# indutny/elliptic

Hardware: NVIDIA H100
Metric: secp256k1 ECDSA verifies/sec (higher is better)
Workload: dtype u32 limbs (integer, exact)

## Files before the change

elliptic_b200/csrc/eb200.cu:

```cuda
#include <cuda_runtime.h>
#include <stdio.h>
#include <string.h>
#include <atomic>
#include <condition_variable>
#include <cstdlib>
#include <mutex>
#include <thread>
#include <type_traits>
#include <vector>
#include "../../include/elliptic_b200.h"
#include "ecdsa_k256_body.cuh"
#include "ecdsa_k256_replay.cuh"
#include "ecdsa_sw_replay.cuh"
#include "ecdsa_k256_sign_fast.cuh"
#include "der_sig.cuh"
#include "ecdsa_sw_sign.cuh"
#include "ecdsa_k256_sign.cuh"
#include "ecdsa_sw_body.cuh"
#include "ed25519_body.cuh"
#include "ed25519_ec.cuh"
#include "sw_runtime.cuh"

using namespace eb;

#ifndef EB_VERIFY_BLOCK
#define EB_VERIFY_BLOCK 128
#endif
#ifndef EB_VERIFY_MINBLOCKS
#define EB_VERIFY_MINBLOCKS 3
#endif

__global__ void __launch_bounds__(128) k256_gtab_kernel(u32* gtab) {
  size_t t = (size_t)blockIdx.x * blockDim.x + threadIdx.x;
  if (t >= (size_t)GTAB_WINDOWS * GTAB_ENTRIES) return;
  int j = (int)(t / GTAB_ENTRIES), idx = (int)(t % GTAB_ENTRIES);
  gtab_entry(j, idx, gtab + t * 16);
}

__global__ void __launch_bounds__(128) k256_prep_kernel(size_t N, const uint8_t* __restrict__ e,
                                                        const uint8_t* __restrict__ r,
                                                        const uint8_t* __restrict__ s,
                                                        u32* __restrict__ ws, u32* __restrict__ scratch) {
  size_t tid = (size_t)blockIdx.x * blockDim.x + threadIdx.x;
  size_t T = (size_t)gridDim.x * blockDim.x;
  prep_thread(tid, T, N, e, r, s, ws, scratch);
}

__global__ void __launch_bounds__(EB_VERIFY_BLOCK, EB_VERIFY_MINBLOCKS)
k256_verify_kernel(size_t N, const uint8_t* __restrict__ pub, const uint8_t* __restrict__ r,
                   const u32* __restrict__ ws, const u32* __restrict__ gtab,
                   u32* __restrict__ qtab, const uint8_t* __restrict__ pre, uint8_t* __restrict__ status) {
  size_t i = (size_t)blockIdx.x * blockDim.x + threadIdx.x;
  if (i >= N) return;
  if (pre && pre[i]) { status[i] = pre[i]; return; }
  status[i] = verify_item(i, N, pub, r, ws, gtab, qtab);
}

__global__ void __launch_bounds__(128) k256_prep_recover_kernel(size_t N, const uint8_t* __restrict__ e,
                                                                const uint8_t* __restrict__ r,
                                                                const uint8_t* __restrict__ s,
                                                                u32* __restrict__ ws, u32* __restrict__ scratch) {
  size_t tid = (size_t)blockIdx.x * blockDim.x + threadIdx.x;
  size_t T = (size_t)gridDim.x * blockDim.x;
  prep_thread(tid, T, N, e, r, s, ws, scratch, 1);
}
__global__ void __launch_bounds__(EB_VERIFY_BLOCK, EB_VERIFY_MINBLOCKS)
k256_recover_kernel(size_t N, const uint8_t* __restrict__ r, const uint8_t* __restrict__ recid,
                    const u32* __restrict__ ws, const u32* __restrict__ gtab, u32* __restrict__ qtab,
                    uint8_t* __restrict__ out, uint8_t* __restrict__ status) {
  size_t i = (size_t)blockIdx.x * blockDim.x + threadIdx.x;
  if (i >= N) return;
  status[i] = recover_item(i, N, r, recid, ws, gtab, qtab, out);
}

__global__ void __launch_bounds__(128)
k256_sign_nonce_kernel(size_t N, const uint8_t* __restrict__ e, const uint8_t* __restrict__ priv,
                       const u32* __restrict__ gtab, u32* __restrict__ ws, uint8_t* __restrict__ status,
                       const uint8_t* __restrict__ kgiven) {
  size_t i = (size_t)blockIdx.x * blockDim.x + threadIdx.x;
  if (i < N) k256_sign_nonce_item(i, N, e, priv, gtab, ws, status, kgiven);
}
__global__ void __launch_bounds__(128)
k256_sign_finish_kernel(size_t N, const uint8_t* __restrict__ e, const uint8_t* __restrict__ priv, u32 canonical,
                        const u32* __restrict__ ws, u32* __restrict__ scratch, uint8_t* __restrict__ r,
                        uint8_t* __restrict__ s, uint8_t* __restrict__ recid, uint8_t* __restrict__ status) {
  size_t tid = (size_t)blockIdx.x * blockDim.x + threadIdx.x;
  size_t T = (size_t)gridDim.x * blockDim.x;
  k256_sign_finish_thread(tid, T, N, e, priv, canonical, ws, scratch, r, s, recid, status);
}
__global__ void __launch_bounds__(128)
k256_sign_slow_kernel(size_t N, const uint8_t* __restrict__ e, const uint8_t* __restrict__ priv, u32 canonical,
                      const u32* __restrict__ gtab, uint8_t* __restrict__ r, uint8_t* __restrict__ s,
                      uint8_t* __restrict__ recid, uint8_t* __restrict__ status) {
  size_t i = (size_t)blockIdx.x * blockDim.x + threadIdx.x;
  if (i >= N || status[i] != ST_NEEDS_HOST) return;
  status[i] = k256_sign_item(i, e, priv, canonical, gtab, r, s, recid);
}

__global__ void __launch_bounds__(128) k256_replay_tab_kernel(u32* tab) {
  int t = blockIdx.x * blockDim.x + threadIdx.x;
  if (t < 2 * REPLAY_NAF_PTS) rp_tab_entry(t, tab + 16 * t);
}
__global__ void __launch_bounds__(128)
k256_replay_kernel(size_t N, const uint8_t* __restrict__ e, const uint8_t* __restrict__ r, const uint8_t* __restrict__ s,
                   const uint8_t* __restrict__ pub, const u32* __restrict__ tab, uint8_t* __restrict__ status) {
  size_t i = (size_t)blockIdx.x * blockDim.x + threadIdx.x;
  if (i >= N || status[i] != ST_NEEDS_HOST) return;
  status[i] = rp_verify_item(i, e, r, s, pub, tab);
}

__global__ void __launch_bounds__(128)
k256_prep_scalars_kernel(size_t N, const uint8_t* __restrict__ k1, const uint8_t* __restrict__ k2, u32* __restrict__ ws) {
  size_t i = (size_t)blockIdx.x * blockDim.x + threadIdx.x;
  if (i < N) prep_scalars_item(i, N, k1, k2, ws);
}
__global__ void __launch_bounds__(EB_VERIFY_BLOCK, EB_VERIFY_MINBLOCKS)
k256_mul_add_kernel(size_t N, const uint8_t* __restrict__ pts, const u32* __restrict__ ws, const u32* __restrict__ gtab,
                    u32* __restrict__ qtab, uint8_t* __restrict__ out, uint8_t* __restrict__ status) {
  size_t i = (size_t)blockIdx.x * blockDim.x + threadIdx.x;
  if (i >= N) return;
  status[i] = mul_add_item(i, N, pts, ws, gtab, qtab, out);
}
__global__ void __launch_bounds__(128)
k256_mul_add_replay_kernel(size_t N, const uint8_t* __restrict__ k1, const uint8_t* __restrict__ k2,
                           const uint8_t* __restrict__ pts, const u32* __restrict__ tab, uint8_t* __restrict__ out,
                           uint8_t* __restrict__ status) {
  size_t i = (size_t)blockIdx.x * blockDim.x + threadIdx.x;
  if (i >= N || status[i] != ST_NEEDS_HOST) return;
  status[i] = rp_mul_add_item(i, k1, k2, pts, tab, out);
}
__global__ void __launch_bounds__(128)
k256_mul_g_kernel(size_t N, const uint8_t* __restrict__ k, const u32* __restrict__ gtab, uint8_t* __restrict__ out,
                  uint8_t* __restrict__ status) {
  size_t i = (size_t)blockIdx.x * blockDim.x + threadIdx.x;
  if (i >= N) return;
  status[i] = k256_mul_g_item(i, k, gtab, out);
}

__global__ void status_map_kernel(size_t N, uint8_t* __restrict__ status, uint8_t from, uint8_t to) {
  size_t i = (size_t)blockIdx.x * blockDim.x + threadIdx.x;
  if (i < N && status[i] == from) status[i] = to;
}

__global__ void __launch_bounds__(128)
der_decode_kernel(size_t N, u32 len, const uint8_t* __restrict__ der, const unsigned long long* __restrict__ off,
                  uint8_t* __restrict__ r, uint8_t* __restrict__ s, uint8_t* __restrict__ pre, int pre_valid) {
  size_t i = (size_t)blockIdx.x * blockDim.x + threadIdx.x;
  if (i >= N) return;
  bool ok = der_import(der + off[i], (size_t)(off[i + 1] - off[i]), len, r + (size_t)len * i, s + (size_t)len * i);
  uint8_t st = pre_valid ? pre[i] : 0;
  if (!st && !ok) st = ST_THROW_SIG_FORMAT;
  pre[i] = st;
}

__global__ void __launch_bounds__(128) k256_decode_pub_kernel(size_t N, const uint8_t* __restrict__ in, u32 fmt,
                                                              uint8_t* __restrict__ xy, uint8_t* __restrict__ pre) {
  size_t i = (size_t)blockIdx.x * blockDim.x + threadIdx.x;
  if (i >= N) return;
  uint8_t st = 0;
  if (fmt == EB200_PUB_SEC1_65) {
    const uint8_t* p = in + 65 * i;
    uint8_t tag = p[0];
    if (tag != 4 && tag != 6 && tag != 7) st = ST_THROW_POINT_FORMAT;
    else if ((tag == 6 && (p[64] & 1)) || (tag == 7 && !(p[64] & 1))) st = ST_THROW_ASSERT;
    for (int k = 0; k < 64; k++) xy[64 * i + k] = p[1 + k];
  } else {
    const uint8_t* p = in + 33 * i;
    uint8_t tag = p[0];
    if (tag != 2 && tag != 3) st = ST_THROW_POINT_FORMAT;
    fe x = fe_from_be(p + 1);
    fe seven = fe_zero(); seven.v[0] = 7;
    fe y2 = fe_add(fe_mul(fe_sqr(x), x), seven);
    fe y = fe_sqrt_candidate(y2);
    if (!st && !fe_eq(fe_sqr(y), y2)) st = ST_THROW_INVALID_POINT;
    y = fe_normalize(y);
    bool odd = tag == 3;
    if (((y.v[0] & 1) != 0) != odd) y = fe_normalize(fe_neg(y));
    x = fe_normalize(x);
    store_be<8>(xy + 64 * i, x.v);
    store_be<8>(xy + 64 * i + 32, y.v);
  }
  pre[i] = st;
// ... 1674 lines not shown
```

elliptic_b200/csrc/ecdsa_k256_body.cuh:

```cuda
#pragma once
#include "ge_k256.cuh"
#include "sc_k256.cuh"
#ifndef EB_K256_FQ
#define EB_K256_FQ 0
#endif
#include "gq_k256.cuh"

namespace eb {

enum : uint8_t {
  ST_FALSE = 0, ST_TRUE = 1, ST_THROW_INVALID_POINT = 2, ST_THROW_NOT_VALIDATED = 3,
  ST_NEEDS_HOST = 4, ST_THROW_ASSERT = 5, ST_THROW_POINT_FORMAT = 6, ST_INFINITY = 7, ST_THROW_SECOND_KEY = 8, ST_THROW_SIG_FORMAT = 9,
};

constexpr int PREP_WORDS = 19;
constexpr u32 FL_INVALID = 1, FL_NEGG = 2, FL_NEG1 = 4, FL_NEG2 = 8, FL_NOG = 16;
constexpr int PREP_BATCH = 16;
constexpr int QTAB_ENTRIES = 8;
#if EB_K256_FQ
constexpr int QTAB_WORDS = QTABQ_WORDS;
#else
constexpr int QTAB_WORDS = QTAB_ENTRIES * 24;
#endif
#ifndef EB_GW
#define EB_GW 20
#endif
constexpr int GTAB_W = EB_GW;
constexpr int GTAB_WINDOWS = (255 + GTAB_W - 1) / GTAB_W;
constexpr int GTAB_ENTRIES = 1 << (GTAB_W - 1);
static_assert(255 - GTAB_W * (GTAB_WINDOWS - 1) <= GTAB_W - 1, "top digit 2m+1 must stay below 2^W");

struct madd_out { ge_jac r; fe h; };

#if defined(__CUDACC__)
#define EB_FN __host__ __device__ __noinline__
#else
#define EB_FN
#endif

EB_FN ge_jac jac_dbl(ge_jac p) { return jac_dbl_inl(p); }
EB_FN ge_jac jac_madd(ge_jac a, ge_aff p) { return jac_madd_inl(a, p); }

EB_HD madd_out jac_madd_h(const ge_jac& a, const ge_aff& p) {
  madd_out o;
  fe z2 = fe_sqr(a.z);
  fe u2 = fe_mul(p.x, z2);
  fe s2 = fe_mul(fe_mul(p.y, z2), a.z);
  fe h = fe_sub(a.x, u2);
  fe rr = fe_sub(a.y, s2);
  fe h2 = fe_sqr(h);
  fe h3 = fe_mul(h2, h);
  fe v = fe_mul(a.x, h2);
  o.r.x = fe_sub(fe_sub(fe_add(fe_sqr(rr), h3), v), v);
  o.r.y = fe_sub(fe_mul(rr, fe_sub(v, o.r.x)), fe_mul(a.y, h3));
  o.r.z = fe_mul(a.z, h);
  o.h = h;
  return o;
}

EB_HD fe fe_beta() {
  fe b;
  const u32 v[8] = {0x719501eeu, 0xc1396c28u, 0x12f58995u, 0x9cf04975u, 0xac3434e9u, 0x6e64479eu, 0x657c0710u, 0x7ae96a2bu};
  for (int i = 0; i < 8; i++) b.v[i] = v[i];
  return b;
}

EB_HD ge_aff k256_G() {
  ge_aff g;
  const u32 x[8] = {0x16f81798u, 0x59f2815bu, 0x2dce28d9u, 0x029bfcdbu, 0xce870b07u, 0x55a06295u, 0xf9dcbbacu, 0x79be667eu};
  const u32 y[8] = {0xfb10d4b8u, 0x9c47d08fu, 0xa6855419u, 0xfd17b448u, 0x0e1108a8u, 0x5da4fbfcu, 0x26a3c465u, 0x483ada77u};
  for (int i = 0; i < 8; i++) { g.x.v[i] = x[i]; g.y.v[i] = y[i]; }
  return g;
}

EB_HD void gtab_entry(int j, int idx, u32* out16) {
  ge_jac b = jac_from_aff(k256_G());
  for (int k = 0; k < GTAB_W * j; k++) b = jac_dbl(b);
  ge_aff base = jac_to_aff(b);
  u32 s = 2 * idx + 1;
  ge_jac acc = jac_infinity();
  for (int k = GTAB_W - 1; k >= 0; k--) {
    acc = jac_dbl(acc);
    if ((s >> k) & 1) acc = jac_madd(acc, base);
  }
  ge_aff r = jac_to_aff(acc);
  r.x = fe_normalize(r.x);
  r.y = fe_normalize(r.y);
  for (int i = 0; i < 8; i++) { out16[i] = r.x.v[i]; out16[8 + i] = r.y.v[i]; }
}

EB_HD void prep_store(size_t i, size_t N, u32* u1, const u32* u2, u32 flags, u32* ws) {
  u32 nn[8];
  K256N::n(nn);
  if ((u1[0] & 1) == 0) {
    sub_n<8>(u1, nn, u1);
    flags |= FL_NEGG;
  }
  u32 m1[5], m2[5];
  bool n1, n2;
  glv_split_odd(u2, m1, &n1, m2, &n2);
  if (n1) flags |= FL_NEG1;
  if (n2) flags |= FL_NEG2;
  for (int w = 0; w < 8; w++) {
    u32 hi = (w < 7) ? u1[w + 1] : 0;
    ws[(size_t)w * N + i] = (u1[w] >> 1) | (hi << 31);
  }
  for (int w = 0; w < 5; w++) {
    ws[(size_t)(8 + w) * N + i] = m1[w];
    ws[(size_t)(13 + w) * N + i] = m2[w];
  }
  ws[(size_t)18 * N + i] = flags;
}

EB_HD void prep_thread(size_t tid, size_t T, size_t N, const uint8_t* e, const uint8_t* r,
                       const uint8_t* s, u32* ws, u32* scratch, int mode = 0) {
  u32 R2[8], one[8], nn[8];
  K256N::r2(R2); K256N::r1(one); K256N::n(nn);
  u32 prod[8];
  copy_n<8>(prod, one);
  u32 invalid_mask = 0;
  int cnt = 0;
  for (int j = 0; j < PREP_BATCH; j++) {
    size_t i = tid + (size_t)j * T;
    if (i >= N) break;
    cnt = j + 1;
    u32 sv[8], rv[8];
    load_be<8>(sv, s + 32 * i);
    load_be<8>(rv, r + 32 * i);
    bool ok = sc_in_range(sv) && sc_in_range(rv);
    u32 sm[8];
    if (mode == 1) {
      sc_mont_mul(sm, rv, R2);
      ok = !is_zero_n<8>(sm);
    } else {
      sc_mont_mul(sm, sv, R2);
    }
    if (!ok) invalid_mask |= 1u << j;
    cmov_n<8>(sm, one, !ok);
    for (int w = 0; w < 8; w++) scratch[(size_t)w * N + i] = prod[w];
    u32 t[8];
    sc_mont_mul(t, prod, sm);
    copy_n<8>(prod, t);
  }
  if (cnt == 0) return;
  u32 inv[8];
  sc_mont_inv(inv, prod);
  for (int j = cnt - 1; j >= 0; j--) {
    size_t i = tid + (size_t)j * T;
    bool ok = !((invalid_mask >> j) & 1);
    u32 sv[8], rv[8], ev[8], sm[8], pre[8], sinv[8], t[8];
    load_be<8>(sv, s + 32 * i);
    load_be<8>(rv, r + 32 * i);
    sc_mont_mul(sm, mode == 1 ? rv : sv, R2);
    cmov_n<8>(sm, one, !ok);
    for (int w = 0; w < 8; w++) pre[w] = scratch[(size_t)w * N + i];
    sc_mont_mul(sinv, inv, pre);
    sc_mont_mul(t, inv, sm);
    copy_n<8>(inv, t);
    u32 flags = (ok || mode == 1) ? 0 : FL_INVALID;
    load_be<8>(ev, e + 32 * i);
    u32 u1[8], u2[8];
    if (mode == 1) {
      u32 zero8[8] = {0, 0, 0, 0, 0, 0, 0, 0};
      cmov_n<8>(sinv, zero8, !ok);
      sc_mont_mul(u1, ev, sinv);
      if (!is_zero_n<8>(u1)) sub_n<8>(u1, nn, u1);
      sc_mont_mul(u2, sv, sinv);
    } else {
      sc_mont_mul(u1, ev, sinv);
      sc_mont_mul(u2, rv, sinv);
    }
    prep_store(i, N, u1, u2, flags, ws);
  }
}

EB_HD void prep_scalars_item(size_t i, size_t N, const uint8_t* k1, const uint8_t* k2, u32* ws) {
  u32 nn[8], u1[8] = {0, 0, 0, 0, 0, 0, 0, 0}, u2[8];
  K256N::n(nn);
  u32 flags = 0;
  if (k1) {
    load_be<8>(u1, k1 + 32 * i);
    if (geq_n<8>(u1, nn)) sub_n<8>(u1, u1, nn);
  } else {
    flags |= FL_NOG;
  }
  load_be<8>(u2, k2 + 32 * i);
  if (geq_n<8>(u2, nn)) sub_n<8>(u2, u2, nn);
  prep_store(i, N, u1, u2, flags, ws);
}

EB_HD void store_fe(u32* dst, const fe& a) { for (int i = 0; i < 8; i++) dst[i] = a.v[i]; }
EB_HD fe load_fe(const u32* src) { fe a; for (int i = 0; i < 8; i++) a.v[i] = src[i]; return a; }

#if EB_K256_FQ
EB_HD ge_jac k256_dsm(size_t i, size_t N, const ge_aff& Q, u32 flags, const u32* ws, const u32* gtab, u32* qtab) {
  u32* tab = qtab + (size_t)i * QTAB_WORDS;
  fqk<1> zglobal;
  {
    gq_jac Qj; Qj.x = fqk_from_fe(Q.x); Qj.y = fqk_from_fe(Q.y); Qj.z = fqk_one();
    gq_jac D = gq_dbl(Qj);
    fqk<1> C2 = fq_sqr(D.z);
    fqk<1> C3 = fq_mul(C2, D.z);
    gq_jac P;
    P.x = fq_mul(Qj.x, C2);
    P.y = fq_mul(Qj.y, C3);
    P.z = fqk_one();
    fq_store12(tab + 0, P.x); fq_store12(tab + FQ_PAD, P.y);
    for (int k = 1; k < QTAB_ENTRIES; k++) {
      gq_madd_out o = gq_madd_h(P, D.x, D.y);
      P = o.r;
      u32* e = tab + QTABQ_ENTRY_WORDS * k;
      fq_store12(e, P.x); fq_store12(e + FQ_PAD, P.y);
      fq_store12(e + 2 * FQ_PAD, o.h);
    }
    zglobal = fq_mul(P.z, D.z);
    const fqk<1> beta = fqk_from_fe(fe_beta());
    fqk<1> zs = fqk_one();
    for (int k = QTAB_ENTRIES - 1; k >= 0; k--) {
      u32* e = tab + QTABQ_ENTRY_WORDS * k;
      fqk<1> X = fq_load12(e), Y = fq_load12(e + FQ_PAD);
      fqk<1> hk = fqk_one();
      if (k > 0) hk = fq_load12(e + 2 * FQ_PAD);
      if (k < QTAB_ENTRIES - 1) {
        fqk<1> zs2 = fq_sqr(zs);
        fqk<1> zs3 = fq_mul(zs2, zs);
        X = fq_mul(X, zs2);
        Y = fq_mul(Y, zs3);
        fq_store12(e, X); fq_store12(e + FQ_PAD, Y);
      }
      fq_store12(e + 2 * FQ_PAD, fq_mul(X, beta));
      zs = fq_mul(zs, hk);
    }
  }

  gq_jac acc;
  acc.x = fqk_one(); acc.y = fqk_one(); acc.z = fqk_zero();
  for (int w = 32; w >= 0; w--) {
    if (w != 32)
      for (int d = 0; d < 4; d++) acc = gq_dbl(acc);
    for (int h = 0; h < 2; h++) {
      u32 word = ws[(size_t)((h ? 13 : 8) + (w >> 3)) * N + i];
      u32 nib = (word >> (4 * (w & 7))) & 15;
      bool dneg = (w != 32) && (nib < 8);
      u32 idx = (w == 32) ? (nib & 7) : (dneg ? 7 - nib : nib - 8);
      bool neg = dneg != (((flags & (h ? FL_NEG2 : FL_NEG1)) != 0));
      const u32* e = tab + QTABQ_ENTRY_WORDS * idx;
      gq_aff P;
      P.x = fq_load12(e + (h ? 2 * FQ_PAD : 0));
      P.y = fq_cneg(fq_load12(e + FQ_PAD), neg);
      if (w == 32 && h == 0) acc = gq_from_aff(P);
      else acc = gq_madd(acc, P);
    }
  }
  acc.z = fq_mul(acc.z, zglobal);

  if (!(flags & FL_NOG)) {
    for (int j = 0; j < GTAB_WINDOWS; j++) {
      const int pos = GTAB_W * j;
      u32 lo = ws[(size_t)(pos >> 5) * N + i];
      u32 hi = ((pos >> 5) < 7) ? ws[(size_t)((pos >> 5) + 1) * N + i] : 0u;
      u64 both = ((u64)hi << 32) | lo;
      u32 chunk = (u32)(both >> (pos & 31)) & ((1u << GTAB_W) - 1);
      const u32 half = 1u << (GTAB_W - 1);
      bool dneg = (j != GTAB_WINDOWS - 1) && (chunk < half);
      u32 idx = (j == GTAB_WINDOWS - 1) ? (chunk & (half - 1)) : (dneg ? half - 1 - chunk : chunk - half);
      bool neg = dneg != ((flags & FL_NEGG) != 0);
      const u32* ent = gtab + ((size_t)j * GTAB_ENTRIES + idx) * 16;
      gq_aff P;
      P.x = fqk_from_fe(load_fe(ent));
      P.y = fq_cneg(fqk_from_fe(load_fe(ent + 8)), neg);
      acc = gq_madd(acc, P);
    }
  }
  return gq_to_jac(acc);
}
#else
EB_HD ge_jac k256_dsm(size_t i, size_t N, const ge_aff& Q, u32 flags, const u32* ws, const u32* gtab, u32* qtab) {
  u32* tab = qtab + (size_t)i * QTAB_WORDS;
  fe zglobal;
  {
    ge_jac D = jac_dbl(jac_from_aff(Q));
    fe C2 = fe_sqr(D.z);
    fe C3 = fe_mul(C2, D.z);
    ge_aff Dp; Dp.x = D.x; Dp.y = D.y;
    ge_jac P;
    P.x = fe_mul(Q.x, C2);
    P.y = fe_mul(Q.y, C3);
    P.z = fe_one();
    store_fe(tab + 0, P.x); store_fe(tab + 8, P.y);
    for (int k = 1; k < QTAB_ENTRIES; k++) {
      madd_out o = jac_madd_h(P, Dp);
      P = o.r;
      store_fe(tab + 24 * k, P.x); store_fe(tab + 24 * k + 8, P.y);
      store_fe(tab + 24 * k + 16, o.h);
    }
    zglobal = fe_mul(P.z, D.z);
    fe beta = fe_beta();
    fe zs = fe_one();
    for (int k = QTAB_ENTRIES - 1; k >= 0; k--) {
      fe X = load_fe(tab + 24 * k), Y = load_fe(tab + 24 * k + 8);
      fe hk = fe_one();
      if (k > 0) hk = load_fe(tab + 24 * k + 16);
      if (k < QTAB_ENTRIES - 1) {
        fe zs2 = fe_sqr(zs);
        fe zs3 = fe_mul(zs2, zs);
        X = fe_mul(X, zs2);
        Y = fe_mul(Y, zs3);
        store_fe(tab + 24 * k, X); store_fe(tab + 24 * k + 8, Y);
      }
      store_fe(tab + 24 * k + 16, fe_mul(X, beta));
      zs = fe_mul(zs, hk);
    }
  }

  ge_jac acc = jac_infinity();
  for (int w = 32; w >= 0; w--) {
    if (w != 32)
      for (int d = 0; d < 4; d++) acc = jac_dbl(acc);
    for (int h = 0; h < 2; h++) {
      u32 word = ws[(size_t)((h ? 13 : 8) + (w >> 3)) * N + i];
      u32 nib = (word >> (4 * (w & 7))) & 15;
      bool dneg = (w != 32) && (nib < 8);
      u32 idx = (w == 32) ? (nib & 7) : (dneg ? 7 - nib : nib - 8);
      bool neg = dneg != (((flags & (h ? FL_NEG2 : FL_NEG1)) != 0));
      ge_aff P;
      P.x = load_fe(tab + 24 * idx + (h ? 16 : 0));
      P.y = load_fe(tab + 24 * idx + 8);
      P = aff_neg_if(P, neg);
      if (w == 32 && h == 0) acc = jac_from_aff(P);
      else acc = jac_madd(acc, P);
    }
  }
  acc.z = fe_mul(acc.z, zglobal);

  if (flags & FL_NOG) return acc;
  for (int j = 0; j < GTAB_WINDOWS; j++) {
    const int pos = GTAB_W * j;
    u32 lo = ws[(size_t)(pos >> 5) * N + i];
    u32 hi = ((pos >> 5) < 7) ? ws[(size_t)((pos >> 5) + 1) * N + i] : 0u;
    u64 both = ((u64)hi << 32) | lo;
    u32 chunk = (u32)(both >> (pos & 31)) & ((1u << GTAB_W) - 1);
    const u32 half = 1u << (GTAB_W - 1);
    bool dneg = (j != GTAB_WINDOWS - 1) && (chunk < half);
    u32 idx = (j == GTAB_WINDOWS - 1) ? (chunk & (half - 1)) : (dneg ? half - 1 - chunk : chunk - half);
    bool neg = dneg != ((flags & FL_NEGG) != 0);
    const u32* ent = gtab + ((size_t)j * GTAB_ENTRIES + idx) * 16;
    ge_aff P;
    P.x = load_fe(ent);
    P.y = load_fe(ent + 8);
    acc = jac_madd(acc, aff_neg_if(P, neg));
  }
  return acc;
}

#endif

EB_HD uint8_t verify_item(size_t i, size_t N, const uint8_t* pub, const uint8_t* r,
                          const u32* ws, const u32* gtab, u32* qtab) {
  u32 flags = ws[(size_t)18 * N + i];
  if (flags & FL_INVALID) return ST_FALSE;
  ge_aff Q;
  Q.x = fe_from_be(pub + 64 * i);
  Q.y = fe_from_be(pub + 64 * i + 32);
  if (!aff_on_curve(Q)) return ST_NEEDS_HOST;
  ge_jac acc = k256_dsm(i, N, Q, flags, ws, gtab, qtab);

  if (fe_is_zero(acc.z)) return ST_FALSE;
  fe z2 = fe_sqr(acc.z);
  fe rf = fe_from_be(r + 32 * i);
  if (fe_eq(acc.x, fe_mul(rf, z2))) return ST_TRUE;
  const u32 pmn[8] = {0x2fc9baeeu, 0x402da172u, 0x50b75fc4u, 0x45512319u, 0x00000001u, 0, 0, 0};
  if (!geq_n<8>(rf.v, pmn)) {
    u32 nn[8]; K256N::n(nn);
    fe rn;
    add_n<8>(rn.v, rf.v, nn);
    if (fe_eq(acc.x, fe_mul(rn, z2))) return ST_TRUE;
  }
  return ST_FALSE;
}

EB_HD uint8_t recover_item(size_t i, size_t N, const uint8_t* r, const uint8_t* recid,
                           const u32* ws, const u32* gtab, u32* qtab, uint8_t* out) {
  for (int b = 0; b < 64; b++) out[64 * i + b] = 0;
  u32 j = recid[i];
  bool odd = j & 1, second = (j >> 1) & 1;
  u32 rv[8];
  load_be<8>(rv, r + 32 * i);
  const u32 pmn[8] = {0x2fc9baeeu, 0x402da172u, 0x50b75fc4u, 0x45512319u, 0x00000001u, 0, 0, 0};
  if (second && geq_n<8>(rv, pmn)) return ST_THROW_SECOND_KEY;
  fe x; copy_n<8>(x.v, rv);
  if (second) { u32 nn[8]; K256N::n(nn); add_n<8>(x.v, rv, nn); }
  fe seven = fe_zero(); seven.v[0] = 7;
  fe y2 = fe_add(fe_mul(fe_sqr(x), x), seven);
  fe y = fe_sqrt_candidate(y2);
  if (!fe_eq(fe_sqr(y), y2)) return ST_THROW_INVALID_POINT;
  if (fe_is_odd(y) != odd) y = fe_neg(y);
  ge_aff R; R.x = x; R.y = y;
  u32 flags = ws[(size_t)18 * N + i];
  ge_jac acc = k256_dsm(i, N, R, flags, ws, gtab, qtab);
  if (fe_is_zero(acc.z)) return ST_INFINITY;
  ge_aff q = jac_to_aff(acc);
  fe qx = fe_normalize(q.x), qy = fe_normalize(q.y);
  store_be<8>(out + 64 * i, qx.v);
  store_be<8>(out + 64 * i + 32, qy.v);
  return ST_TRUE;
}

EB_HD uint8_t mul_add_item(size_t i, size_t N, const uint8_t* pts, const u32* ws, const u32* gtab, u32* qtab,
                           uint8_t* out) {
  for (int b = 0; b < 64; b++) out[64 * i + b] = 0;
  ge_aff P;
  P.x = fe_from_be(pts + 64 * i);
  P.y = fe_from_be(pts + 64 * i + 32);
  if (!aff_on_curve(P)) return ST_NEEDS_HOST;
  u32 flags = ws[(size_t)18 * N + i];
  ge_jac acc = k256_dsm(i, N, P, flags, ws, gtab, qtab);
  if (fe_is_zero(acc.z)) return ST_INFINITY;
  ge_aff q = jac_to_aff(acc);
  fe qx = fe_normalize(q.x), qy = fe_normalize(q.y);
  store_be<8>(out + 64 * i, qx.v);
  store_be<8>(out + 64 * i + 32, qy.v);
  return ST_TRUE;
}

}
```

elliptic_b200/csrc/ge_k256.cuh:

```cuda
#pragma once
#include "fe_k256.cuh"

namespace eb {

struct ge_aff { fe x, y; };
struct ge_jac { fe x, y, z; };

#if defined(__CUDACC__)
#define EB_NOINLINE __noinline__
#else
#define EB_NOINLINE
#endif

EB_HD ge_jac jac_infinity() {
  ge_jac r; r.x = fe_one(); r.y = fe_one(); r.z = fe_zero(); return r;
}
EB_HD bool jac_is_infinity(const ge_jac& a) { return fe_is_zero(a.z); }

EB_HD ge_jac jac_from_aff(const ge_aff& p) {
  ge_jac r; r.x = p.x; r.y = p.y; r.z = fe_one(); return r;
}

EB_HD ge_jac jac_dbl_inl(const ge_jac& p) {
  fe A = fe_sqr_hot(p.x);
  fe B = fe_sqr_hot(p.y);
  fe C = fe_sqr_hot(B);
  fe t = fe_add(p.x, B);
  t = fe_sqr_hot(t);
  t = fe_sub(t, A);
  t = fe_sub(t, C);
  fe D = fe_dbl(t);
  fe E = fe_mul_small(A, 3);
  fe F = fe_sqr_hot(E);
  ge_jac r;
  r.x = fe_sub(F, fe_dbl(D));
  fe C8 = fe_mul_small(C, 8);
#if EB_FE_MUL2
  fe2 m = fe_mul2(E, fe_sub(D, r.x), p.y, p.z);
  r.y = fe_sub(m.a, C8);
  r.z = fe_dbl(m.b);
#else
  r.y = fe_sub(fe_mul(E, fe_sub(D, r.x)), C8);
  r.z = fe_dbl(fe_mul(p.y, p.z));
#endif
  return r;
}

EB_HD ge_jac jac_dbl_aff(const ge_aff& p) { return jac_dbl_inl(jac_from_aff(p)); }

EB_HD ge_jac jac_madd_inl(const ge_jac& a, const ge_aff& p) {
  fe z2 = fe_sqr_hot(a.z);
#if EB_FE_MUL2
  fe2 m1 = fe_mul2(p.x, z2, p.y, z2);
  fe h = fe_sub(a.x, m1.a);
  fe2 m2 = fe_mul2(m1.b, a.z, a.z, h);
  fe rr = fe_sub(a.y, m2.a);
  fe h2 = fe_sqr_hot(h);
  fe2 m3 = fe_mul2(h2, h, a.x, h2);
  fe h3 = m3.a, v = m3.b;
  ge_jac r;
  r.x = fe_sub(fe_sub(fe_add(fe_sqr_hot(rr), h3), v), v);
  fe2 m4 = fe_mul2(rr, fe_sub(v, r.x), a.y, h3);
  r.y = fe_sub(m4.a, m4.b);
  r.z = m2.b;
#else
  fe u2 = fe_mul(p.x, z2);
  fe s2 = fe_mul(fe_mul(p.y, z2), a.z);
  fe h = fe_sub(a.x, u2);
  fe rr = fe_sub(a.y, s2);
  fe h2 = fe_sqr_hot(h);
  fe h3 = fe_mul(h2, h);
  fe v = fe_mul(a.x, h2);
  ge_jac r;
  r.x = fe_sub(fe_sub(fe_add(fe_sqr_hot(rr), h3), v), v);
  r.y = fe_sub(fe_mul(rr, fe_sub(v, r.x)), fe_mul(a.y, h3));
  r.z = fe_mul(a.z, h);
#endif
  if (fe_is_zero(r.z)) {
    if (fe_is_zero(a.z)) return jac_from_aff(p);
    if (fe_is_zero(rr)) return jac_dbl_inl(a);
    return jac_infinity();
  }
  return r;
}

EB_HD ge_jac jac_add_inl(const ge_jac& a, const ge_jac& b) {
  if (fe_is_zero(a.z)) return b;
  if (fe_is_zero(b.z)) return a;
  fe bz2 = fe_sqr(b.z);
  fe az2 = fe_sqr(a.z);
  fe u1 = fe_mul(a.x, bz2);
  fe u2 = fe_mul(b.x, az2);
  fe s1 = fe_mul(a.y, fe_mul(bz2, b.z));
  fe s2 = fe_mul(b.y, fe_mul(az2, a.z));
  fe h = fe_sub(u1, u2);
  fe rr = fe_sub(s1, s2);
  if (fe_is_zero(h)) {
    if (fe_is_zero(rr)) return jac_dbl_inl(a);
    return jac_infinity();
  }
  fe h2 = fe_sqr(h);
  fe h3 = fe_mul(h2, h);
  fe v = fe_mul(u1, h2);
  ge_jac r;
  r.x = fe_sub(fe_sub(fe_add(fe_sqr(rr), h3), v), v);
  r.y = fe_sub(fe_mul(rr, fe_sub(v, r.x)), fe_mul(s1, h3));
  r.z = fe_mul(fe_mul(a.z, b.z), h);
  return r;
}

EB_HD ge_aff aff_neg_if(const ge_aff& p, bool neg) {
  ge_aff r; r.x = p.x; r.y = fe_cmov(p.y, fe_neg(p.y), neg); return r;
}

EB_HD bool aff_on_curve(const ge_aff& p) {
  fe x3 = fe_mul(fe_sqr(p.x), p.x);
  fe seven = fe_zero(); seven.v[0] = 7;
  return fe_eq(fe_sqr(p.y), fe_add(x3, seven));
}

EB_HD ge_aff jac_to_aff(const ge_jac& a) {
  fe zi = fe_inv(a.z);
  fe zi2 = fe_sqr(zi);
  ge_aff r;
  r.x = fe_mul(a.x, zi2);
  r.y = fe_mul(fe_mul(a.y, zi2), zi);
  return r;
}

}
```

elliptic_b200/csrc/sc_k256.cuh:

```cuda
#pragma once
#include "limbs.cuh"
#include "fp_mont.cuh"

namespace eb {

struct K256N {
  static EB_HD void n(u32* r) {
    const u32 v[8] = {0xd0364141u, 0xbfd25e8cu, 0xaf48a03bu, 0xbaaedce6u, 0xfffffffeu, 0xffffffffu, 0xffffffffu, 0xffffffffu};
    for (int i = 0; i < 8; i++) r[i] = v[i];
  }
  static EB_HD void r2(u32* r) {
    const u32 v[8] = {0x67d7d140u, 0x896cf214u, 0x0e7cf878u, 0x741496c2u, 0x5bcd07c6u, 0xe697f5e4u, 0x81c69bc5u, 0x9d671cd5u};
    for (int i = 0; i < 8; i++) r[i] = v[i];
  }
  static EB_HD void r1(u32* r) {
    const u32 v[8] = {0x2fc9bebfu, 0x402da173u, 0x50b75fc4u, 0x45512319u, 0x00000001u, 0, 0, 0};
    for (int i = 0; i < 8; i++) r[i] = v[i];
  }
  static constexpr u32 n0inv = 0x5588b13fu;
};

struct K256_FN {
  static constexpr int N = 8;
  static constexpr u32 n0inv = K256N::n0inv;
  static EB_HD void mod(u32* r) { K256N::n(r); }
  static EB_HD void r1(u32* r) { K256N::r1(r); }
  static EB_HD void r2(u32* r) { K256N::r2(r); }
};

EB_HD void sc_mont_mul(u32* r, const u32* a, const u32* b) {
#if defined(__CUDA_ARCH__)
  typedef Fp<K256_FN> S;
  S::fe x, y;
#pragma unroll
  for (int i = 0; i < 8; i++) { x.v[i] = a[i]; y.v[i] = b[i]; }
  S::fe z = S::mul(x, y);
#pragma unroll
  for (int i = 0; i < 8; i++) r[i] = z.v[i];
  return;
#endif
  u32 n[8]; K256N::n(n);
  u32 t[10];
#pragma unroll
  for (int i = 0; i < 10; i++) t[i] = 0;
#pragma unroll
  for (int i = 0; i < 8; i++) {
    u64 c = 0;
#pragma unroll
    for (int j = 0; j < 8; j++) {
      c += (u64)a[j] * b[i] + t[j];
      t[j] = (u32)c; c >>= 32;
    }
    c += t[8];
    t[8] = (u32)c; t[9] = (u32)(c >> 32);
    u32 m = t[0] * K256N::n0inv;
    c = (u64)m * n[0] + t[0];
    c >>= 32;
#pragma unroll
    for (int j = 1; j < 8; j++) {
      c += (u64)m * n[j] + t[j];
      t[j - 1] = (u32)c; c >>= 32;
    }
    c += t[8];
    t[7] = (u32)c;
    t[8] = t[9] + (u32)(c >> 32);
    t[9] = 0;
  }
  u32 d[8];
  u32 bw = sub_n<8>(d, t, n);
  bool ge = t[8] != 0 || bw == 0;
#pragma unroll
  for (int i = 0; i < 8; i++) r[i] = ge ? d[i] : t[i];
}

EB_HD void sc_mont_inv(u32* r, const u32* a) {
  const u32 e[8] = {0xd036413fu, 0xbfd25e8cu, 0xaf48a03bu, 0xbaaedce6u, 0xfffffffeu, 0xffffffffu, 0xffffffffu, 0xffffffffu};
  u32 acc[8], base[8];
  copy_n<8>(base, a);
  copy_n<8>(acc, a);
  for (int i = 254; i >= 0; i--) {
    u32 t[8];
    sc_mont_mul(t, acc, acc);
    copy_n<8>(acc, t);
    if ((e[i >> 5] >> (i & 31)) & 1) {
      sc_mont_mul(t, acc, base);
      copy_n<8>(acc, t);
    }
  }
  copy_n<8>(r, acc);
}

EB_HD bool sc_in_range(const u32* a) {
  u32 n[8]; K256N::n(n);
  return !is_zero_n<8>(a) && !geq_n<8>(a, n);
}

EB_HD void neg256(u32* r, const u32* a) {
  u32 z[8] = {0, 0, 0, 0, 0, 0, 0, 0};
  sub_n<8>(r, z, a);
}

EB_HD void glv_split_odd(const u32* k, u32* m1, bool* neg1, u32* m2, bool* neg2) {
  const u32 g1[8] = {0x45dbb031u, 0xe893209au, 0x71e8ca7fu, 0x3daa8a14u, 0x9284eb15u, 0xe86c90e4u, 0xa7d46bcdu, 0x3086d221u};
  const u32 g2[8] = {0x8ac47f71u, 0x1571b4aeu, 0x9df506c6u, 0x221208acu, 0x0abfe4c4u, 0x6f547fa9u, 0x010e8828u, 0xe4437ed6u};
  const u32 a1[8] = {0x9284eb15u, 0xe86c90e4u, 0xa7d46bcdu, 0x3086d221u, 0, 0, 0, 0};
  const u32 mb1[8] = {0x0abfe4c3u, 0x6f547fa9u, 0x010e8828u, 0xe4437ed6u, 0, 0, 0, 0};
  const u32 a2[8] = {0x9d44cfd8u, 0x57c1108du, 0xa8e2f3f6u, 0x14ca50f7u, 0x00000001u, 0, 0, 0};
  const u32 b2[8] = {0x9284eb15u, 0xe86c90e4u, 0xa7d46bcdu, 0x3086d221u, 0, 0, 0, 0};
  u32 t[16], c1[4], c2[4];
  const u32 half[4] = {0, 0, 0, 0x80000000u};
  mul_rect<8, 8>(t, k, g1);
  {
    u32 cy = add_n<4>(t + 8, t + 8, half);
    u32 one[4] = {cy, 0, 0, 0};
    add_n<4>(c1, t + 12, one);
  }
  mul_rect<8, 8>(t, k, g2);
  {
    u32 cy = add_n<4>(t + 8, t + 8, half);
    u32 one[4] = {cy, 0, 0, 0};
    add_n<4>(c2, t + 12, one);
  }
  u32 p[9], k1[8], k2[8], q[8];
  mul_rect<4, 4>(p, c1, a1);
  sub_n<8>(k1, k, p);
  mul_rect<5, 4>(p, a2, c2);
  sub_n<8>(k1, k1, p);
  mul_rect<4, 4>(k2, c1, mb1);
  mul_rect<4, 4>(q, c2, b2);
  sub_n<8>(k2, k2, q);
  bool k1neg = (k1[7] >> 31) != 0;
  if ((k1[0] & 1) == 0) {
    if (!k1neg) { sub_n<8>(k1, k1, a1); add_n<8>(k2, k2, mb1); }
    else        { add_n<8>(k1, k1, a1); sub_n<8>(k2, k2, mb1); }
    k1neg = (k1[7] >> 31) != 0;
  }
  if ((k2[0] & 1) == 0) {
    if (!k1neg) { sub_n<8>(k1, k1, a2); sub_n<8>(k2, k2, b2); }
    else        { add_n<8>(k1, k1, a2); add_n<8>(k2, k2, b2); }
  }
  *neg1 = (k1[7] >> 31) != 0;
  *neg2 = (k2[7] >> 31) != 0;
  u32 a[8];
  neg256(a, k1); cmov_n<8>(k1, a, *neg1);
  neg256(a, k2); cmov_n<8>(k2, a, *neg2);
#pragma unroll
  for (int i = 0; i < 5; i++) {
    m1[i] = (k1[i] >> 1) | (k1[i + 1] << 31);
    m2[i] = (k2[i] >> 1) | (k2[i + 1] << 31);
  }
}

}
```

Measured before the change: 41.06 million.

## Use co-Z table build, addition-chain scalar inverse, inlined field ops, occupancy 4

Replaces the mixed-add precompute chain for the Q table with co-Z additions that skip Z tracking, and derives the global Z from accumulated h values. Swaps the square-and-multiply scalar inversion for an addition chain with 2-bit windowed digits, cutting the number of multiplies. Lets jac_dbl inline its field multiplies through a template switch, and raises the launch-bounds minimum blocks from 3 to 4. The higher occupancy target squeezes registers and may cause spills, and inlining grows code size.

```diff
diff --git a/elliptic_b200/csrc/eb200.cu b/elliptic_b200/csrc/eb200.cu
--- a/elliptic_b200/csrc/eb200.cu
+++ b/elliptic_b200/csrc/eb200.cu
@@ -27,7 +27,7 @@
 #define EB_VERIFY_BLOCK 128
 #endif
 #ifndef EB_VERIFY_MINBLOCKS
-#define EB_VERIFY_MINBLOCKS 3
+#define EB_VERIFY_MINBLOCKS 4
 #endif
 
 __global__ void __launch_bounds__(128) k256_gtab_kernel(u32* gtab) {
diff --git a/elliptic_b200/csrc/ecdsa_k256_body.cuh b/elliptic_b200/csrc/ecdsa_k256_body.cuh
--- a/elliptic_b200/csrc/ecdsa_k256_body.cuh
+++ b/elliptic_b200/csrc/ecdsa_k256_body.cuh
@@ -32,15 +32,6 @@
 
 struct madd_out { ge_jac r; fe h; };
 
-#if defined(__CUDACC__)
-#define EB_FN __host__ __device__ __noinline__
-#else
-#define EB_FN
-#endif
-
-EB_FN ge_jac jac_dbl(ge_jac p) { return jac_dbl_inl(p); }
-EB_FN ge_jac jac_madd(ge_jac a, ge_aff p) { return jac_madd_inl(a, p); }
-
 EB_HD madd_out jac_madd_h(const ge_jac& a, const ge_aff& p) {
   madd_out o;
   fe z2 = fe_sqr(a.z);
@@ -56,6 +47,21 @@
   o.r.z = fe_mul(a.z, h);
   o.h = h;
   return o;
+}
+
+EB_HD fe jac_zaddu_h(ge_aff& P, ge_aff& D) {
+  fe h = fe_sub(P.x, D.x);
+  fe rr = fe_sub(P.y, D.y);
+  fe A = fe_sqr(h);
+  fe x1 = fe_mul(D.x, A);
+  fe B = fe_mul(P.x, A);
+  fe y1 = fe_mul(D.y, fe_sub(B, x1));
+  fe x3 = fe_sub(fe_sub(fe_sqr(rr), x1), B);
+  P.y = fe_sub(fe_mul(rr, fe_sub(x1, x3)), y1);
+  P.x = x3;
+  D.x = x1;
+  D.y = y1;
+  return h;
 }
 
 EB_HD fe fe_beta() {
@@ -275,43 +281,43 @@
   return gq_to_jac(acc);
 }
 #else
+EB_HD fe k256_qtab_build(const ge_aff& Q, u32* tab) {
+  ge_jac D = jac_dbl(jac_from_aff(Q));
+  fe C2 = fe_sqr(D.z);
+  fe C3 = fe_mul(C2, D.z);
+  ge_aff Dp; Dp.x = D.x; Dp.y = D.y;
+  ge_aff P;
+  P.x = fe_mul(Q.x, C2);
+  P.y = fe_mul(Q.y, C3);
+  store_fe(tab + 0, P.x); store_fe(tab + 8, P.y);
+  for (int k = 1; k < QTAB_ENTRIES; k++) {
+    fe h = jac_zaddu_h(P, Dp);
+    store_fe(tab + 24 * k, P.x); store_fe(tab + 24 * k + 8, P.y);
+    store_fe(tab + 24 * k + 16, h);
+  }
+  fe beta = fe_beta();
+  fe zs = fe_one();
+  for (int k = QTAB_ENTRIES - 1; k >= 0; k--) {
+    fe X = load_fe(tab + 24 * k), Y = load_fe(tab + 24 * k + 8);
+    fe hk = fe_one();
+    if (k > 0) hk = load_fe(tab + 24 * k + 16);
+    if (k < QTAB_ENTRIES - 1) {
+      fe zs2 = fe_sqr(zs);
+      fe zs3 = fe_mul(zs2, zs);
+      X = fe_mul(X, zs2);
+      Y = fe_mul(Y, zs3);
+      store_fe(tab + 24 * k, X); store_fe(tab + 24 * k + 8, Y);
+    }
+    store_fe(tab + 24 * k + 16, fe_mul(X, beta));
+    if (k == QTAB_ENTRIES - 1) zs = hk;
+    else if (k > 0) zs = fe_mul(zs, hk);
+  }
+  return fe_mul(zs, D.z);
+}
+
 EB_HD ge_jac k256_dsm(size_t i, size_t N, const ge_aff& Q, u32 flags, const u32* ws, const u32* gtab, u32* qtab) {
   u32* tab = qtab + (size_t)i * QTAB_WORDS;
-  fe zglobal;
-  {
-    ge_jac D = jac_dbl(jac_from_aff(Q));
-    fe C2 = fe_sqr(D.z);
-    fe C3 = fe_mul(C2, D.z);
-    ge_aff Dp; Dp.x = D.x; Dp.y = D.y;
-    ge_jac P;
-    P.x = fe_mul(Q.x, C2);
-    P.y = fe_mul(Q.y, C3);
-    P.z = fe_one();
-    store_fe(tab + 0, P.x); store_fe(tab + 8, P.y);
-    for (int k = 1; k < QTAB_ENTRIES; k++) {
-      madd_out o = jac_madd_h(P, Dp);
-      P = o.r;
-      store_fe(tab + 24 * k, P.x); store_fe(tab + 24 * k + 8, P.y);
-      store_fe(tab + 24 * k + 16, o.h);
-    }
-    zglobal = fe_mul(P.z, D.z);
-    fe beta = fe_beta();
-    fe zs = fe_one();
-    for (int k = QTAB_ENTRIES - 1; k >= 0; k--) {
-      fe X = load_fe(tab + 24 * k), Y = load_fe(tab + 24 * k + 8);
-      fe hk = fe_one();
-      if (k > 0) hk = load_fe(tab + 24 * k + 16);
-      if (k < QTAB_ENTRIES - 1) {
-        fe zs2 = fe_sqr(zs);
-        fe zs3 = fe_mul(zs2, zs);
-        X = fe_mul(X, zs2);
-        Y = fe_mul(Y, zs3);
-        store_fe(tab + 24 * k, X); store_fe(tab + 24 * k + 8, Y);
-      }
-      store_fe(tab + 24 * k + 16, fe_mul(X, beta));
-      zs = fe_mul(zs, hk);
-    }
-  }
+  fe zglobal = k256_qtab_build(Q, tab);
 
   ge_jac acc = jac_infinity();
   for (int w = 32; w >= 0; w--) {
diff --git a/elliptic_b200/csrc/ge_k256.cuh b/elliptic_b200/csrc/ge_k256.cuh
--- a/elliptic_b200/csrc/ge_k256.cuh
+++ b/elliptic_b200/csrc/ge_k256.cuh
@@ -21,17 +21,30 @@
   ge_jac r; r.x = p.x; r.y = p.y; r.z = fe_one(); return r;
 }
 
+#ifndef EB_GL_INLINE
+#define EB_GL_INLINE 1
+#endif
+template <bool INL> EB_HD fe gl_mul(const fe& a, const fe& b) {
+  if (INL) return fe_mul_inl(a, b);
+  return fe_mul(a, b);
+}
+template <bool INL> EB_HD fe gl_sqr(const fe& a) {
+  if (INL) return fe_sqr_inl(a);
+  return fe_sqr_hot(a);
+}
+
+template <bool INL = false>
 EB_HD ge_jac jac_dbl_inl(const ge_jac& p) {
-  fe A = fe_sqr_hot(p.x);
-  fe B = fe_sqr_hot(p.y);
-  fe C = fe_sqr_hot(B);
+  fe A = gl_sqr<INL>(p.x);
+  fe B = gl_sqr<INL>(p.y);
+  fe C = gl_sqr<INL>(B);
   fe t = fe_add(p.x, B);
-  t = fe_sqr_hot(t);
+  t = gl_sqr<INL>(t);
   t = fe_sub(t, A);
   t = fe_sub(t, C);
   fe D = fe_dbl(t);
   fe E = fe_mul_small(A, 3);
-  fe F = fe_sqr_hot(E);
+  fe F = gl_sqr<INL>(E);
   ge_jac r;
   r.x = fe_sub(F, fe_dbl(D));
   fe C8 = fe_mul_small(C, 8);
@@ -40,16 +53,24 @@
   r.y = fe_sub(m.a, C8);
   r.z = fe_dbl(m.b);
 #else
-  r.y = fe_sub(fe_mul(E, fe_sub(D, r.x)), C8);
-  r.z = fe_dbl(fe_mul(p.y, p.z));
+  r.y = fe_sub(gl_mul<INL>(E, fe_sub(D, r.x)), C8);
+  r.z = fe_dbl(gl_mul<INL>(p.y, p.z));
 #endif
   return r;
 }
 
+#if defined(__CUDACC__)
+#define EB_FN __host__ __device__ __noinline__
+#else
+#define EB_FN
+#endif
+EB_FN ge_jac jac_dbl(ge_jac p) { return jac_dbl_inl<(EB_GL_INLINE >= 1)>(p); }
+
 EB_HD ge_jac jac_dbl_aff(const ge_aff& p) { return jac_dbl_inl(jac_from_aff(p)); }
 
+template <bool INL = false>
 EB_HD ge_jac jac_madd_inl(const ge_jac& a, const ge_aff& p) {
-  fe z2 = fe_sqr_hot(a.z);
+  fe z2 = gl_sqr<INL>(a.z);
 #if EB_FE_MUL2
   fe2 m1 = fe_mul2(p.x, z2, p.y, z2);
   fe h = fe_sub(a.x, m1.a);
@@ -64,25 +85,30 @@
   r.y = fe_sub(m4.a, m4.b);
   r.z = m2.b;
 #else
-  fe u2 = fe_mul(p.x, z2);
-  fe s2 = fe_mul(fe_mul(p.y, z2), a.z);
+  fe u2 = gl_mul<INL>(p.x, z2);
+  fe s2 = gl_mul<INL>(gl_mul<INL>(p.y, z2), a.z);
   fe h = fe_sub(a.x, u2);
   fe rr = fe_sub(a.y, s2);
-  fe h2 = fe_sqr_hot(h);
-  fe h3 = fe_mul(h2, h);
-  fe v = fe_mul(a.x, h2);
+  fe h2 = gl_sqr<INL>(h);
+  fe h3 = gl_mul<INL>(h2, h);
+  fe v = gl_mul<INL>(a.x, h2);
   ge_jac r;
-  r.x = fe_sub(fe_sub(fe_add(fe_sqr_hot(rr), h3), v), v);
-  r.y = fe_sub(fe_mul(rr, fe_sub(v, r.x)), fe_mul(a.y, h3));
-  r.z = fe_mul(a.z, h);
+  r.x = fe_sub(fe_sub(fe_add(gl_sqr<INL>(rr), h3), v), v);
+  r.y = fe_sub(gl_mul<INL>(rr, fe_sub(v, r.x)), gl_mul<INL>(a.y, h3));
+  r.z = gl_mul<INL>(a.z, h);
 #endif
   if (fe_is_zero(r.z)) {
     if (fe_is_zero(a.z)) return jac_from_aff(p);
-    if (fe_is_zero(rr)) return jac_dbl_inl(a);
+    if (fe_is_zero(rr)) {
+      if (INL) return jac_dbl(a);
+      return jac_dbl_inl(a);
+    }
     return jac_infinity();
   }
   return r;
 }
+
+EB_FN ge_jac jac_madd(ge_jac a, ge_aff p) { return jac_madd_inl<(EB_GL_INLINE >= 2)>(a, p); }
 
 EB_HD ge_jac jac_add_inl(const ge_jac& a, const ge_jac& b) {
   if (fe_is_zero(a.z)) return b;
diff --git a/elliptic_b200/csrc/sc_k256.cuh b/elliptic_b200/csrc/sc_k256.cuh
--- a/elliptic_b200/csrc/sc_k256.cuh
+++ b/elliptic_b200/csrc/sc_k256.cuh
@@ -73,7 +73,52 @@
   for (int i = 0; i < 8; i++) r[i] = ge ? d[i] : t[i];
 }
 
+EB_HD void sc_mont_sqr_n(u32* x, int k) {
+  for (int i = 0; i < k; i++) {
+    u32 t[8];
+    sc_mont_mul(t, x, x);
+    copy_n<8>(x, t);
+  }
+}
+
+EB_HD void sc_mont_sqr_n_mul(u32* x, int k, const u32* y) {
+  u32 t[8];
+  sc_mont_sqr_n(x, k);
+  sc_mont_mul(t, x, y);
+  copy_n<8>(x, t);
+}
+
 EB_HD void sc_mont_inv(u32* r, const u32* a) {
+  u32 a2[8], x2[8], a5[8], x3[8], x6[8], x12[8], x24[8], x48[8], x[8];
+  sc_mont_mul(a2, a, a);
+  sc_mont_mul(x2, a2, a);
+  sc_mont_mul(a5, x2, a2);
+  sc_mont_mul(x3, a5, a2);
+  copy_n<8>(x6, x3);   sc_mont_sqr_n_mul(x6, 3, x3);
+  copy_n<8>(x12, x6);  sc_mont_sqr_n_mul(x12, 6, x6);
+  copy_n<8>(x24, x12); sc_mont_sqr_n_mul(x24, 12, x12);
+  copy_n<8>(x48, x24); sc_mont_sqr_n_mul(x48, 24, x24);
+  copy_n<8>(x, x48);
+  sc_mont_sqr_n_mul(x, 48, x48);
+  sc_mont_sqr_n_mul(x, 24, x24);
+  sc_mont_sqr_n_mul(x, 6, x6);
+  sc_mont_sqr_n_mul(x, 1, a);
+  const u64 W0 = 0x914d744d29244a4ull, W1 = 0x92cf4d3a9838f4ull, W2 = 0xd36025150b3943ull, W3 = 0x33d46ull;
+  for (int s = 0; s < 33; s++) {
+    u64 w = s < 10 ? W0 : s < 20 ? W1 : s < 30 ? W2 : W3;
+    u32 c = (u32)(w >> (6 * (s % 10))) & 63;
+    u32 d = c >> 4;
+    u32 m[8];
+    copy_n<8>(m, a);
+    cmov_n<8>(m, x2, d == 1);
+    cmov_n<8>(m, a5, d == 2);
+    cmov_n<8>(m, x3, d == 3);
+    sc_mont_sqr_n_mul(x, (int)(c & 15), m);
+  }
+  copy_n<8>(r, x);
+}
+
+EB_HD void sc_mont_inv_ladder(u32* r, const u32* a) {
   const u32 e[8] = {0xd036413fu, 0xbfd25e8cu, 0xaf48a03bu, 0xbaaedce6u, 0xfffffffeu, 0xffffffffu, 0xffffffffu, 0xffffffffu};
   u32 acc[8], base[8];
   copy_n<8>(base, a);
```

New measurement: 42.35 million (median of 6 runs). 3.1% higher.

## Use co-Z table build, cheaper doubling constants, early madd checks, raise min blocks

Applied to the files above, without the earlier changes.

The per-signature Q table build moves into a noinline function that uses co-Z style additions, avoiding a full Jacobian mixed add per entry. Doubling now uses additions and doublings instead of small-constant multiplies. The mixed add checks for infinity and h==0 up front rather than after computing z. Minimum blocks per SM in launch bounds goes from 3 to 4, which tightens the register budget and may cause spills.

```diff
diff --git a/elliptic_b200/csrc/eb200.cu b/elliptic_b200/csrc/eb200.cu
--- a/elliptic_b200/csrc/eb200.cu
+++ b/elliptic_b200/csrc/eb200.cu
@@ -27,7 +27,7 @@
 #define EB_VERIFY_BLOCK 128
 #endif
 #ifndef EB_VERIFY_MINBLOCKS
-#define EB_VERIFY_MINBLOCKS 3
+#define EB_VERIFY_MINBLOCKS 4
 #endif
 
 __global__ void __launch_bounds__(128) k256_gtab_kernel(u32* gtab) {
diff --git a/elliptic_b200/csrc/ecdsa_k256_body.cuh b/elliptic_b200/csrc/ecdsa_k256_body.cuh
--- a/elliptic_b200/csrc/ecdsa_k256_body.cuh
+++ b/elliptic_b200/csrc/ecdsa_k256_body.cuh
@@ -30,8 +30,6 @@
 constexpr int GTAB_ENTRIES = 1 << (GTAB_W - 1);
 static_assert(255 - GTAB_W * (GTAB_WINDOWS - 1) <= GTAB_W - 1, "top digit 2m+1 must stay below 2^W");
 
-struct madd_out { ge_jac r; fe h; };
-
 #if defined(__CUDACC__)
 #define EB_FN __host__ __device__ __noinline__
 #else
@@ -40,23 +38,6 @@
 
 EB_FN ge_jac jac_dbl(ge_jac p) { return jac_dbl_inl(p); }
 EB_FN ge_jac jac_madd(ge_jac a, ge_aff p) { return jac_madd_inl(a, p); }
-
-EB_HD madd_out jac_madd_h(const ge_jac& a, const ge_aff& p) {
-  madd_out o;
-  fe z2 = fe_sqr(a.z);
-  fe u2 = fe_mul(p.x, z2);
-  fe s2 = fe_mul(fe_mul(p.y, z2), a.z);
-  fe h = fe_sub(a.x, u2);
-  fe rr = fe_sub(a.y, s2);
-  fe h2 = fe_sqr(h);
-  fe h3 = fe_mul(h2, h);
-  fe v = fe_mul(a.x, h2);
-  o.r.x = fe_sub(fe_sub(fe_add(fe_sqr(rr), h3), v), v);
-  o.r.y = fe_sub(fe_mul(rr, fe_sub(v, o.r.x)), fe_mul(a.y, h3));
-  o.r.z = fe_mul(a.z, h);
-  o.h = h;
-  return o;
-}
 
 EB_HD fe fe_beta() {
   fe b;
@@ -192,6 +173,43 @@
 EB_HD void store_fe(u32* dst, const fe& a) { for (int i = 0; i < 8; i++) dst[i] = a.v[i]; }
 EB_HD fe load_fe(const u32* src) { fe a; for (int i = 0; i < 8; i++) a.v[i] = src[i]; return a; }
 
+#if !EB_K256_FQ
+EB_FN fe k256_qtab_build(ge_aff Q, u32* tab) {
+  ge_jac D = jac_dbl(jac_from_aff(Q));
+  fe C2 = fe_sqr(D.z);
+  fe px = fe_mul(Q.x, C2), py = fe_mul(Q.y, fe_mul(C2, D.z));
+  fe dx = D.x, dy = D.y;
+  store_fe(tab + 0, px); store_fe(tab + 8, py);
+  for (int k = 1; k < QTAB_ENTRIES; k++) {
+    fe h = fe_sub(dx, px);
+    fe c = fe_sqr(h);
+    fe w1 = fe_mul(dx, c), w2 = fe_mul(px, c);
+    fe ry = fe_sub(dy, py);
+    dy = fe_mul(dy, fe_sub(w1, w2));
+    dx = w1;
+    px = fe_sub(fe_sub(fe_sqr(ry), w1), w2);
+    py = fe_sub(fe_mul(ry, fe_sub(w1, px)), dy);
+    store_fe(tab + 24 * k, px); store_fe(tab + 24 * k + 8, py);
+    store_fe(tab + 24 * k + 16, h);
+  }
+  fe beta = fe_beta();
+  fe zs = fe_one();
+  for (int k = QTAB_ENTRIES - 1; k >= 0; k--) {
+    fe X = load_fe(tab + 24 * k), Y = load_fe(tab + 24 * k + 8);
+    if (k < QTAB_ENTRIES - 1) {
+      fe zs2 = fe_sqr(zs);
+      fe zs3 = fe_mul(zs2, zs);
+      X = fe_mul(X, zs2);
+      Y = fe_mul(Y, zs3);
+      store_fe(tab + 24 * k, X); store_fe(tab + 24 * k + 8, Y);
+    }
+    if (k > 0) zs = fe_mul(zs, load_fe(tab + 24 * k + 16));
+    store_fe(tab + 24 * k + 16, fe_mul(X, beta));
+  }
+  return fe_mul(zs, D.z);
+}
+#endif
+
 #if EB_K256_FQ
 EB_HD ge_jac k256_dsm(size_t i, size_t N, const ge_aff& Q, u32 flags, const u32* ws, const u32* gtab, u32* qtab) {
   u32* tab = qtab + (size_t)i * QTAB_WORDS;
@@ -277,41 +295,7 @@
 #else
 EB_HD ge_jac k256_dsm(size_t i, size_t N, const ge_aff& Q, u32 flags, const u32* ws, const u32* gtab, u32* qtab) {
   u32* tab = qtab + (size_t)i * QTAB_WORDS;
-  fe zglobal;
-  {
-    ge_jac D = jac_dbl(jac_from_aff(Q));
-    fe C2 = fe_sqr(D.z);
-    fe C3 = fe_mul(C2, D.z);
-    ge_aff Dp; Dp.x = D.x; Dp.y = D.y;
-    ge_jac P;
-    P.x = fe_mul(Q.x, C2);
-    P.y = fe_mul(Q.y, C3);
-    P.z = fe_one();
-    store_fe(tab + 0, P.x); store_fe(tab + 8, P.y);
-    for (int k = 1; k < QTAB_ENTRIES; k++) {
-      madd_out o = jac_madd_h(P, Dp);
-      P = o.r;
-      store_fe(tab + 24 * k, P.x); store_fe(tab + 24 * k + 8, P.y);
-      store_fe(tab + 24 * k + 16, o.h);
-    }
-    zglobal = fe_mul(P.z, D.z);
-    fe beta = fe_beta();
-    fe zs = fe_one();
-    for (int k = QTAB_ENTRIES - 1; k >= 0; k--) {
-      fe X = load_fe(tab + 24 * k), Y = load_fe(tab + 24 * k + 8);
-      fe hk = fe_one();
-      if (k > 0) hk = load_fe(tab + 24 * k + 16);
-      if (k < QTAB_ENTRIES - 1) {
-        fe zs2 = fe_sqr(zs);
-        fe zs3 = fe_mul(zs2, zs);
-        X = fe_mul(X, zs2);
-        Y = fe_mul(Y, zs3);
-        store_fe(tab + 24 * k, X); store_fe(tab + 24 * k + 8, Y);
-      }
-      store_fe(tab + 24 * k + 16, fe_mul(X, beta));
-      zs = fe_mul(zs, hk);
-    }
-  }
+  fe zglobal = k256_qtab_build(Q, tab);
 
   ge_jac acc = jac_infinity();
   for (int w = 32; w >= 0; w--) {
diff --git a/elliptic_b200/csrc/ge_k256.cuh b/elliptic_b200/csrc/ge_k256.cuh
--- a/elliptic_b200/csrc/ge_k256.cuh
+++ b/elliptic_b200/csrc/ge_k256.cuh
@@ -30,11 +30,11 @@
   t = fe_sub(t, A);
   t = fe_sub(t, C);
   fe D = fe_dbl(t);
-  fe E = fe_mul_small(A, 3);
+  fe E = fe_add(fe_dbl(A), A);
   fe F = fe_sqr_hot(E);
   ge_jac r;
   r.x = fe_sub(F, fe_dbl(D));
-  fe C8 = fe_mul_small(C, 8);
+  fe C8 = fe_dbl(fe_dbl(fe_dbl(C)));
 #if EB_FE_MUL2
   fe2 m = fe_mul2(E, fe_sub(D, r.x), p.y, p.z);
   r.y = fe_sub(m.a, C8);
@@ -49,12 +49,25 @@
 EB_HD ge_jac jac_dbl_aff(const ge_aff& p) { return jac_dbl_inl(jac_from_aff(p)); }
 
 EB_HD ge_jac jac_madd_inl(const ge_jac& a, const ge_aff& p) {
+  if (fe_is_zero(a.z)) return jac_from_aff(p);
   fe z2 = fe_sqr_hot(a.z);
 #if EB_FE_MUL2
   fe2 m1 = fe_mul2(p.x, z2, p.y, z2);
   fe h = fe_sub(a.x, m1.a);
   fe2 m2 = fe_mul2(m1.b, a.z, a.z, h);
   fe rr = fe_sub(a.y, m2.a);
+  fe z3 = m2.b;
+#else
+  fe u2 = fe_mul(p.x, z2);
+  fe s2 = fe_mul(fe_mul(p.y, z2), a.z);
+  fe h = fe_sub(a.x, u2);
+  fe rr = fe_sub(a.y, s2);
+#endif
+  if (fe_is_zero(h)) {
+    if (fe_is_zero(rr)) return jac_dbl_inl(a);
+    return jac_infinity();
+  }
+#if EB_FE_MUL2
   fe h2 = fe_sqr_hot(h);
   fe2 m3 = fe_mul2(h2, h, a.x, h2);
   fe h3 = m3.a, v = m3.b;
@@ -62,25 +75,17 @@
   r.x = fe_sub(fe_sub(fe_add(fe_sqr_hot(rr), h3), v), v);
   fe2 m4 = fe_mul2(rr, fe_sub(v, r.x), a.y, h3);
   r.y = fe_sub(m4.a, m4.b);
-  r.z = m2.b;
+  r.z = z3;
 #else
-  fe u2 = fe_mul(p.x, z2);
-  fe s2 = fe_mul(fe_mul(p.y, z2), a.z);
-  fe h = fe_sub(a.x, u2);
-  fe rr = fe_sub(a.y, s2);
+  fe z3 = fe_mul(a.z, h);
   fe h2 = fe_sqr_hot(h);
   fe h3 = fe_mul(h2, h);
   fe v = fe_mul(a.x, h2);
   ge_jac r;
   r.x = fe_sub(fe_sub(fe_add(fe_sqr_hot(rr), h3), v), v);
   r.y = fe_sub(fe_mul(rr, fe_sub(v, r.x)), fe_mul(a.y, h3));
-  r.z = fe_mul(a.z, h);
+  r.z = z3;
 #endif
-  if (fe_is_zero(r.z)) {
-    if (fe_is_zero(a.z)) return jac_from_aff(p);
-    if (fe_is_zero(rr)) return jac_dbl_inl(a);
-    return jac_infinity();
-  }
   return r;
 }
 
```

Result: faster. 41.29 million before, 42.40 million after, median of 6 (+2.7%).
